# Kyaw-Thiha/animal-vision

Hardware: AMD Instinct MI355X
Metric: megapixels/sec per-frame pipeline (higher is better)
Workload: dtype f16

## Files before the change

### animal-vision_amd/_lib.py

```python
from __future__ import annotations

import ctypes
import os

_HERE = os.path.dirname(os.path.abspath(__file__))
LIB_PATH = os.path.join(_HERE, "libavx.so")

AVX_OK = 0
AVX_ERR_INVALID, AVX_ERR_NO_DEVICE, AVX_ERR_HIP, AVX_ERR_UNSUPPORTED, AVX_ERR_NOMEM = -1, -2, -3, -4, -5
AVX_COLOR_MATRIX, AVX_COLOR_CAT_MERGE = 0, 1
AVX_POST_NONE, AVX_POST_GAUSS, AVX_POST_ROWGAIN, AVX_POST_STREAK = 0, 1, 2, 3
AVX_MAX_KSIZE = 33
AVX_PIX_FMTS = {"yuv420p": 0, "nv12": 1, "yuv422p": 2, "yuv444p": 3, "gray": 4, "yuv420p10le": 5, "yuv422p10le": 6, "yuv444p10le": 7,
                "p010le": 8}
AVX_TRANSFERS = {"pq": 1, "hlg": 2}
AVX_TONEMAPS = {"clip": 0, "mobius": 1}


class AvxError(RuntimeError):
    def __init__(self, code: int, msg: str):
        super().__init__(f"libavx error {code}: {msg}")
        self.code = code


# ... 253 lines not shown
    "avx_yuv_coefficients_d": (_i, [_i, _i, _i, ctypes.POINTER(ctypes.c_int), ctypes.POINTER(ctypes.c_int)]),
    "avx_yuv_frame_size": (_sz, [_i, _i, _i]),
    "avx_yuv_to_rgb_u8": (_i, [_vp, _i, _vp, _vp, _i, _i, _i, _i, _i, _vp]),
    "avx_rgb_to_yuv_u8": (_i, [_vp, _i, _vp, _vp, _i, _i, _i, _i, _i, _vp]),
    "avx_yuv_hdr_to_rgb_u8": (_i, [_vp, _i, _vp, _vp, _i, _i, _i, _i, _i, _i, ctypes.c_double, ctypes.c_double, _vp]),
    "avx_yuv_to_rgb_scaled_u8": (_i, [_vp, _i, _vp, _vp, _i, _i, _i, _i, _i, _i, _i, _vp]),
    "avx_remap_linear_planes": (_i, [_vp, _vp, _i, _i, _i, _vp, _vp, _vp, ctypes.c_float, _vp]),
    "avx_sobel3_plane": (_i, [_vp, _vp, _i, _i, _vp, _vp, _vp]),
    "avx_mst_gram": (_i, [_vp, _vp, _i, _sz, _i, _i, _vp, _vp, _vp, _vp]),
    "avx_mst_qkv_gram": (_i, [_vp, _vp, _vp, _sz, _i, _vp, _vp, _vp, _vp, _vp]),
    "avx_mst_qkv_gram16": (_i, [_vp, _vp, _vp, _sz, _i, _vp, _vp, _vp, _vp, _vp]),
    "avx_mst_ln_gemm_gelu": (_i, [_vp, _vp, _vp, _vp, ctypes.c_float, _vp, _sz, _i, _vp, _vp]),
    "avx_mst_convt2x2": (_i, [_vp, _vp, _vp, _vp, _vp, _i, _i, _i, _i, _vp]),
    "avx_mst_convt2x2_fuse": (_i, [_vp, _vp, _vp, _vp, _vp, _vp, _vp, _i, _i, _i, _i, _vp]),
    "avx_mst_posemb": (_i, [_vp, _vp, _vp, _vp, _vp, _vp, _vp, _i, _i, _i, _i, _vp]),
    "avx_mst_conv3x3_add": (_i, [_vp, _vp, _vp, _vp, _vp, _i, _i, _i, _i, _vp]),
    "avx_mst_attn_pack": (_i, [_vp, _vp, _vp, _vp, _vp, _vp, _i, _vp, _vp]),
    "avx_mst_rowgemm_add": (_i, [_vp, _vp, _vp, _vp, _vp, _vp, _vp, _sz, _i, _vp]),
    "avx_mst_conv_in_u8": (_i, [_vp, _vp, _i, _i, _i, _i, _i, _i, _vp, _vp, _vp]),
    "avx_mst_conv3x3_lds": (_i, [_vp, _vp, _vp, _vp, _vp, _i, _i, _i, _i, _vp]),
    "avx_mst_down4x4": (_i, [_vp, _vp, _vp, _vp, _i, _i, _i, _i, _vp]),
    "avx_mst_conv3x3_lds_gram": (_i, [_vp, _vp, _vp, _vp, _vp, _i, _i, _i, _vp, _vp, _vp, _vp, _vp]),
    "avx_mst_convt2x2_fuse_gram": (_i, [_vp, _vp, _vp, _vp, _vp, _vp, _vp, _i, _i, _i, _vp, _vp, _vp, _vp, _vp]),
    "avx_mst_attn_pack16": (_i, [_vp, _vp, _vp, _vp, _vp, _vp, _i, _vp, _vp]),
    "avx_mst_attn_pack_mx": (_i, [_vp, _vp, _vp, _vp, _vp, _vp, _i, _vp, _vp]),
    "avx_mst_attn_tail_mx": (_i, [_vp, _vp, _vp, _vp, _vp, _vp, _vp, _vp, _i, _i, _i, _i, _vp]),
    "avx_mst_attn_tail": (_i, [_vp, _vp, _vp, _vp, _vp, _vp, _vp, _vp, _i, _i, _i, _i, _vp]),
    "avx_mst_attn_tail_x": (_i, [_vp, _vp, _vp, _vp, _vp, _vp, _vp, _vp, _i, _i, _i, _i, _vp]),
    "avx_mst_ffn_fused": (_i, [_vp, _vp, _vp, _vp, ctypes.c_float, _vp, _vp, _vp, _vp, _i, _i, _i, _i, _vp]),
    "avx_mst_conv3x3_lds_spectral": (_i, [_vp, _vp, _vp, _vp, _i, _i, _i, _fp, _i, _i, _i, _i, _vp, _vp, ctypes.POINTER(ctypes.c_int), _vp]),
    "avx_mst_ffn_fused_mx": (_i, [_vp, _vp, _vp, _vp, ctypes.c_float, _vp, _vp, _vp, _vp, _i, _i, _i, _i, _vp]),
    "avx_mst_gelu_prescale": (ctypes.c_float, []),
    "avx_mst_tile_order": (_i, [_i, _i, _i, _i, _i, ctypes.POINTER(ctypes.c_longlong), _i, ctypes.POINTER(ctypes.c_int)]),
    "avx_mst_dw_gemm_add": (_i, [_vp, _vp, _vp, _vp, _vp, _vp, _i, _i, _i, _i, _vp]),
    "avx_dwconv3x3_nhwc_add": (_i, [_vp, _vp, _vp, _vp, _i, _i, _i, _i, _i, _vp, _vp, _vp]),
    "avx_dwconv3x3_nhwc": (_i, [_vp, _vp, _vp, _vp, _i, _i, _i, _i, _i, _i, _vp]),
    "avx_layernorm_rows": (_i, [_vp, _vp, _vp, _vp, _vp, _i, _sz, _i, ctypes.c_float, _vp]),
    "avx_layernorm_rows_grouped": (_i, [_vp, _vp, _vp, _vp, _vp, _i, _sz, _i, ctypes.c_float, _i, _i, _vp]),
}
for _name, (_res, _args) in _SIGS.items():
    _fn = getattr(lib, _name)
    _fn.restype = _res
    _fn.argtypes = _args

if lib.avx_abi_version() != 1:
    raise ImportError(f"libavx.so ABI {lib.avx_abi_version()} != 1 expected by this package: rebuild")
```

### animal-vision_amd/csrc/mst_fused.hip

```cpp
#include <hip/hip_fp16.h>

#include <cstdio>
#include <cstdlib>
#include <cstring>

#include "avx_internal.h"
#include "mst_common.h"
#include "mst_tile_order.h"

namespace {

typedef float float4_t __attribute__((ext_vector_type(4)));
#ifndef AVX_FFN32_GM2
#define AVX_FFN32_GM2 1
#endif
constexpr int kFT = 512;
constexpr int TS = 16;
constexpr int HS = TS + 2;
#ifndef AVX_FFN_TH
#define AVX_FFN_TH 16
#endif
constexpr int kFfnTH = AVX_FFN_TH;
static_assert(kFfnTH == 14 || kFfnTH == 16, "FeedForward tile rows");
constexpr int kFfnNGRP = (HS * (kFfnTH + 2) + 31) / 32;
// ... 345 lines not shown
#pragma unroll
                    for (int n = 0; n < NT; ++n)
                        D[n] = mfma16(w2f[n * KS2 + s], bf, D[n]);
                }
            }
        }
        stamp(5);
        {
            const int yo = t.y0 + 2 * w8 + (p >> 4), xo = t.x0 + (p & 15);
            if (2 * w8 < FTH && yo < H && xo < W) {
                const size_t off = ((t.b * H + yo) * (size_t)W + xo) * C + 16 * h + 32 * n0;
#pragma unroll
                for (int n = 0; n < NTW; ++n) {
                    const uint4 xa = reinterpret_cast<const uint4*>(x + off + 32 * n)[0], xb = reinterpret_cast<const uint4*>(x + off + 32 * n)[1];
                    const unsigned xw[8] = {xa.x, xa.y, xa.z, xa.w, xb.x, xb.y, xb.z, xb.w};
                    unsigned ow[8];
#pragma unroll
                    for (int j = 0; j < 8; ++j) {
                        float s0 = D[n][2 * j], s1 = D[n][2 * j + 1];
                        fma_mix_lo(s0, xw[j], 0x3c003c00u); fma_mix_hi(s1, xw[j], 0x3c003c00u);
                        ow[j] = pack_f16(s0, s1);
                    }
                    reinterpret_cast<uint4*>(out + off + 32 * n)[0] = uint4{ow[0], ow[1], ow[2], ow[3]};
                    reinterpret_cast<uint4*>(out + off + 32 * n)[1] = uint4{ow[4], ow[5], ow[6], ow[7]};
                }
            }
        }
        stamp(6);
        if (!ahead.live) break;
        t = tile_at(ahead, TS, FTH);
        ahead.advance();
        if (!PREFETCH) fetch(t);
        layernorm();
    }
    if constexpr (STAMP) {
        if (lane == 0 && stamps)
#pragma unroll
            for (int k = 0; k < 8; ++k) stamps[((size_t)blockIdx.x * NW + wave) * 8 + k] = seg[k];
    }
}


constexpr int VS = TS + 4, MS = TS + 2;

template <int C, int MINW>
__global__ __launch_bounds__(kFT, MINW) void k_mst_attn_tail(const __half* __restrict__ v , const __half* __restrict__ x ,
                                                             const uint4* __restrict__ mpack , const __half* __restrict__ taps1 ,
                                                             const __half* __restrict__ taps2 , const float* __restrict__ bias ,
                                                             __half* __restrict__ out, int B, int H, int W, const uint4* __restrict__ wvpack ) {
    constexpr int NO = C / 8, NS = C / 16, NT = C / 32, PP = C * 2 + 16;
    constexpr int VRP = (VS * PP + 255) / 256 * 256, MRP = VRP;
    constexpr int NFILL = (VS * VS * NO + kFT - 1) / kFT;
    extern __shared__ __align__(16) unsigned char smem[];
    unsigned char* vt = smem;
    unsigned char* mt = vt + (size_t)VS * VRP;
    const bool fromx = wvpack != nullptr;
    __half* t2l = reinterpret_cast<__half*>(mt + (size_t)VS * VRP);
    __half* t1l = t2l + 9 * C;
    float* bl = reinterpret_cast<float*>(t1l + 9 * C);
    const int tid = threadIdx.x, lane = tid & 63, wave = tid >> 6, p = lane & 31, h = lane >> 5;
    for (int i = tid; i < 9 * C; i += kFT) { t2l[i] = taps2[i]; t1l[i] = taps1[i]; }
    for (int i = tid; i < C; i += kFT) bl[i] = bias ? bias[i] : 0.f;
    const int tx = (W + TS - 1) / TS, ty = (H + TS - 1) / TS;
    const int oct = wave % NO, part = wave / NO, nparts = 8 / NO, per = (MS * MS + nparts - 1) / nparts;
    half8_t mf[NT * NS];
#pragma unroll
// ... 930 lines not shown
            unsigned o[8];
#pragma unroll
            for (int vv = 0; vv < 8; ++vv) o[vv] = pack_f16(d[2 * vv], d[2 * vv + 1]);
            reinterpret_cast<uint4*>(out + i * 32 + 16 * h)[0] = uint4{o[0], o[1], o[2], o[3]};
            reinterpret_cast<uint4*>(out + i * 32 + 16 * h)[1] = uint4{o[4], o[5], o[6], o[7]};
        }
    }
}

}

static int ffn_fused_launch(avx_ctx* ctx, const void* x, const float* gamma, const float* beta, float eps, const void* w1pack, const void* taps_9xhid, const void* dwpack,
                            const void* w2pack, void* out, int B, int H, int W, int C, void* stream);

extern "C" float avx_mst_gelu_prescale(void) { return kGeluPrescale; }

extern "C" int avx_mst_tile_order(int frames, int ty, int tx, int nwg, int raster, long long* visit, int steps_cap, int* steps_out) {
    if (frames <= 0 || ty <= 0 || tx <= 0 || nwg <= 0 || (visit && steps_cap <= 0) || (long long)frames * ty * tx > 0x7fffffffll) return AVX_ERR_INVALID;
    int most = 0;
    for (int wg = 0; wg < nwg; ++wg) {
        TileWalk wk;
        wk.init((unsigned)wg, (unsigned)nwg, frames, ty, tx, raster ? AVX_TILE_ORDER_RASTER : AVX_TILE_ORDER_XCD);
        int k = 0;
        for (; wk.live; wk.advance(), ++k)
            if (visit && k < steps_cap) visit[(size_t)wg * steps_cap + k] = ((long long)wk.b * ty + wk.yi) * tx + wk.xi;
        if (visit)
            for (int r = k; r < steps_cap; ++r) visit[(size_t)wg * steps_cap + r] = -1;
        most = k > most ? k : most;
    }
    if (steps_out) *steps_out = most;
    return AVX_OK;
}

extern "C" int avx_mst_ffn_fused(avx_ctx* ctx, const void* x, const float* gamma, const float* beta, float eps, const void* w1pack, const void* taps_9xhid,
                                 const void* w2pack, void* out, int B, int H, int W, int C, void* stream) {
    if (!ctx) return AVX_ERR_INVALID;
    AVX_REQUIRE(ctx, taps_9xhid, "avx_mst_ffn_fused: NULL pointer");
    return ffn_fused_launch(ctx, x, gamma, beta, eps, w1pack, taps_9xhid, nullptr, w2pack, out, B, H, W, C, stream);
}

extern "C" int avx_mst_ffn_fused_mx(avx_ctx* ctx, const void* x, const float* gamma, const float* beta, float eps, const void* w1pack, const void* dwpack,
                                    const void* w2pack, void* out, int B, int H, int W, int C, void* stream) {
    if (!ctx) return AVX_ERR_INVALID;
    AVX_REQUIRE(ctx, dwpack && (((uintptr_t)dwpack) & 15u) == 0, "avx_mst_ffn_fused_mx: dwpack NULL or not 16-byte aligned");
    return ffn_fused_launch(ctx, x, gamma, beta, eps, w1pack, nullptr, dwpack, w2pack, out, B, H, W, C, stream);
}

static int ffn_fused_launch(avx_ctx* ctx, const void* x, const float* gamma, const float* beta, float eps, const void* w1pack, const void* taps_9xhid, const void* dwpack,
                            const void* w2pack, void* out, int B, int H, int W, int C, void* stream) {
    AVX_REQUIRE(ctx, x && gamma && beta && w1pack && w2pack && out && B > 0 && H > 0 && W > 0, "avx_mst_ffn_fused: NULL pointer or empty tensor");
    AVX_REQUIRE(ctx, C == 32 || C == 64 || C == 128, "avx_mst_ffn_fused: C=%d (32, 64 or 128: 31-channel groups stored 32 wide)", C);
    AVX_REQUIRE(ctx, ((((uintptr_t)x | (uintptr_t)w1pack | (uintptr_t)w2pack | (uintptr_t)out | (uintptr_t)taps_9xhid)) & 15u) == 0,
                "avx_mst_ffn_fused: pointers must be 16-byte aligned");
    AVX_REQUIRE(ctx, x != out, "avx_mst_ffn_fused: neighbouring tiles read each other's halo: the output cannot be the input");
    AVX_HIP(ctx, hipSetDevice(ctx->device));
    hipStream_t s = avx_pick_stream(ctx, stream);
    const long total = (long)B * ((H + kFfnTH - 1) / kFfnTH) * ((W + TS - 1) / TS);
    const char* hp = getenv("AVX_MST_FFN_HPASS");
    const bool small = C == 32 && !(hp && atoi(hp) == 128);
    const int hpass = (small || C == 128) ? 64 : 128, hpitch = hpass * 2 + 16, rpitch = (HS * hpitch + 255) / 256 * 256;
    const long cap = (long)ctx->num_cus * (small ? 2 : 1);
    const bool nw16 = C == 64 && dwpack && !(getenv("AVX_MST_FFN_NW") && atoi(getenv("AVX_MST_FFN_NW")) == 8);
    const size_t lds = (size_t)kFfnNGRP * 32 * (C * 2 + 16) + (size_t)(kFfnTH + 2) * rpitch + (dwpack ? 0 : (size_t)9 * 4 * C * 2) + sizeof(float) * 2 * C + (nw16 ? (size_t)(C / 32) * (hpass / 16) * 1024 : 0);
    AVX_REQUIRE(ctx, total <= 0x7fffffffl, "avx_mst_ffn_fused: 2^31 tiles or more");
    const dim3 grid((unsigned)(total < cap ? total : cap));
    const int order = mst_tile_order();
#define AVX_FFN1(CV, HP, MW, DW, NWV)                                                                                                            \
    {                                                                                                                                            \
        auto k = k_mst_ffn_fused<CV, HP, MW, DW, false, NWV>;                                                                                    \
        AVX_HIP(ctx, hipFuncSetAttribute((const void*)k, hipFuncAttributeMaxDynamicSharedMemorySize, (int)lds));                                 \
        hipLaunchKernelGGL(k, grid, dim3(64 * NWV), lds, s, (const __half*)x, gamma, beta, eps, (const uint4*)w1pack, (const __half*)taps_9xhid, \
                           (const uint4*)w2pack, (__half*)out, B, H, W, (const uint4*)dwpack, (unsigned long long*)nullptr, order);              \
    }
#define AVX_FFN(CV, HP, MW) { if (dwpack) AVX_FFN1(CV, HP, MW, true, 8) else AVX_FFN1(CV, HP, MW, false, 8) }
    if (dwpack && getenv("AVX_FFN_STAMPS") && ((C == 32 && small) || C == 64 || C == 128)) {
        unsigned long long* d_st = nullptr;
        const int nwv = nw16 ? 16 : 8;
        const size_t n = (size_t)grid.x * nwv * 8;
        AVX_HIP(ctx, hipMalloc((void**)&d_st, n * sizeof(unsigned long long)));
#define AVX_FFN_ST(CV, HP, MW, NWV)                                                                                                              \
    {                                                                                                                                            \
        auto k = k_mst_ffn_fused<CV, HP, MW, true, true, NWV>;                                                                                   \
        AVX_HIP(ctx, hipFuncSetAttribute((const void*)k, hipFuncAttributeMaxDynamicSharedMemorySize, (int)lds));                                 \
        hipLaunchKernelGGL(k, grid, dim3(64 * NWV), lds, s, (const __half*)x, gamma, beta, eps, (const uint4*)w1pack, (const __half*)taps_9xhid, \
                           (const uint4*)w2pack, (__half*)out, B, H, W, (const uint4*)dwpack, d_st, order);                                      \
    }
        if (C == 32) AVX_FFN_ST(32, 64, 4, 8) else if (nw16) AVX_FFN_ST(64, 128, 1, 16) else if (C == 64) AVX_FFN_ST(64, 128, 2, 8) else AVX_FFN_ST(128, 64, 2, 8)
#undef AVX_FFN_ST
        AVX_HIP(ctx, hipStreamSynchronize(s));
        unsigned long long* h_st = (unsigned long long*)malloc(n * sizeof(unsigned long long));
        AVX_HIP(ctx, hipMemcpy(h_st, d_st, n * sizeof(unsigned long long), hipMemcpyDeviceToHost));
        double tot[8] = {0}, w0[8] = {0}, w7[8] = {0};
        for (size_t i = 0; i < n; ++i) { tot[i & 7] += (double)h_st[i]; if (((i >> 3) % nwv) == 0) w0[i & 7] += (double)h_st[i]; if (((i >> 3) % nwv) == (size_t)nwv - 1) w7[i & 7] += (double)h_st[i]; }
        double all = 0;
        for (int k2 = 0; k2 < 8; ++k2) all += tot[k2];
        fprintf(stderr, "[ffn stamps C=%d] %u blocks x %d waves, mean cycles per wave %.0f; share per segment (all waves | first wave | last wave): ", C, grid.x, nwv, all / (grid.x * (double)nwv));
        const char* nm[8] = {"bar1", "phase1", "bar2", "phase2a", "bar3", "phase2b", "epilogue", "ln+fetch"};
        for (int k2 = 0; k2 < 8; ++k2) fprintf(stderr, "%s %.1f%% | %.1f%% | %.1f%%  ", nm[k2], 100 * tot[k2] / all, 100 * w0[k2] * nwv / all, 100 * w7[k2] * nwv / all);
        fprintf(stderr, "\n");
        free(h_st);
        (void)hipFree(d_st);
    } else if (C == 32 && small) AVX_FFN(32, 64, 4) else if (C == 32) AVX_FFN(32, 128, 2)
    else if (nw16) AVX_FFN1(64, 128, 1, true, 16)
    else if (C == 64) AVX_FFN(64, 128, 2) else AVX_FFN(128, 64, 2)
#undef AVX_FFN
#undef AVX_FFN1
    AVX_HIP(ctx, hipGetLastError());
    return AVX_OK;
}

extern "C" int avx_mst_attn_tail(avx_ctx* ctx, const void* v, const void* x, const void* mpack16, const void* taps1_9xc, const void* taps2_9xc, const float* bias,
                                 void* out, int B, int H, int W, int C, void* stream) {
    if (!ctx) return AVX_ERR_INVALID;
    AVX_REQUIRE(ctx, v && x && mpack16 && taps1_9xc && taps2_9xc && out && B > 0 && H > 0 && W > 0, "avx_mst_attn_tail: NULL pointer or empty tensor");
    AVX_REQUIRE(ctx, C == 32 || C == 64, "avx_mst_attn_tail: C=%d (32 or 64)", C);
    AVX_REQUIRE(ctx, ((((uintptr_t)v | (uintptr_t)x | (uintptr_t)mpack16 | (uintptr_t)out | (uintptr_t)taps1_9xc | (uintptr_t)taps2_9xc)) & 15u) == 0,
                "avx_mst_attn_tail: pointers must be 16-byte aligned");
    AVX_REQUIRE(ctx, v != out, "avx_mst_attn_tail: tiles read their neighbours' rows of v: the output cannot be v (it may be x)");
    AVX_HIP(ctx, hipSetDevice(ctx->device));
    hipStream_t s = avx_pick_stream(ctx, stream);
    if (C == 32) return launch_attn_tail<32, 4>(ctx, v, x, mpack16, taps1_9xc, taps2_9xc, bias, out, B, H, W, s, nullptr);
    return launch_attn_tail<64, 2>(ctx, v, x, mpack16, taps1_9xc, taps2_9xc, bias, out, B, H, W, s, nullptr);
}

extern "C" int avx_mst_attn_tail_x(avx_ctx* ctx, const void* x, const void* wvpack16, const void* mpack16, const void* taps1_9xc, const void* taps2_9xc,
                                   const float* bias, void* out, int B, int H, int W, int C, void* stream) {
    if (!ctx) return AVX_ERR_INVALID;
    AVX_REQUIRE(ctx, x && wvpack16 && mpack16 && taps1_9xc && taps2_9xc && out && B > 0 && H > 0 && W > 0, "avx_mst_attn_tail_x: NULL pointer or empty tensor");
    AVX_REQUIRE(ctx, C == 32 || C == 64, "avx_mst_attn_tail_x: C=%d (32 or 64)", C);
    AVX_REQUIRE(ctx, ((((uintptr_t)x | (uintptr_t)wvpack16 | (uintptr_t)mpack16 | (uintptr_t)out | (uintptr_t)taps1_9xc | (uintptr_t)taps2_9xc)) & 15u) == 0,
                "avx_mst_attn_tail_x: pointers must be 16-byte aligned");
    AVX_REQUIRE(ctx, x != out, "avx_mst_attn_tail_x: tiles read their neighbours' rows of x: the output cannot be x");
    AVX_HIP(ctx, hipSetDevice(ctx->device));
    hipStream_t s = avx_pick_stream(ctx, stream);
// ... 133 lines not shown
```

### animal-vision_amd/csrc/mst_tile_order.h

```cpp
#pragma once

#if defined(__HIP_DEVICE_COMPILE__) && __HIP_DEVICE_COMPILE__
#define AVX_TW_UNI32(v) __builtin_amdgcn_readfirstlane((int)(v))
#else
#define AVX_TW_UNI32(v) ((int)(v))
#endif

enum { AVX_TILE_ORDER_RASTER = 0, AVX_TILE_ORDER_XCD = 1 };
constexpr int kTileXcds = 8;

struct TileWalk {
    int xi, yi, b;
    bool live;
    int x1, w;
    int dx, dy, db;
    int tx, ty, nb;
    unsigned per;
    unsigned pos, end, step, stop;

    __host__ __device__ __forceinline__ void locate() {
        const unsigned qb = (unsigned)tx / (unsigned)nb, rb = (unsigned)tx % (unsigned)nb;
        const unsigned wide = rb * (qb + 1) * per;
        unsigned bstart, wv, x0v;
        if (pos < wide) {
// ... 14 lines not shown
        tx = tx_; ty = ty_; per = (unsigned)frames * (unsigned)ty_;
        const unsigned total = per * (unsigned)tx_;
        if (order == AVX_TILE_ORDER_XCD) {
            const unsigned g = wg % kTileXcds, m = wg / kTileXcds, base = nwg / kTileXcds, rem = nwg % kTileXcds;
            const unsigned cum = g * base + (g < rem ? g : rem), n = base + (g < rem ? 1u : 0u);
            nb = tx_ < kTileXcds ? tx_ : kTileXcds;
            pos = (unsigned)AVX_TW_UNI32((unsigned long long)total * cum / nwg) + m;
            end = (unsigned)AVX_TW_UNI32((unsigned long long)total * (cum + n) / nwg);
            step = n;
        } else {
            nb = 1;
            pos = wg; end = total; step = nwg;
        }
        live = pos < end;
        stop = 0;
        if (live) locate();
    }
    __host__ __device__ __forceinline__ void advance() {
        pos += step;
        if (pos >= stop) {
            live = live && pos < end;
            if (live) locate();
            return;
        }
        xi += dx;
        const int cx = xi >= x1 ? 1 : 0;
        xi -= cx ? w : 0;
        yi += dy + cx;
        const int cy = yi >= ty ? 1 : 0;
        yi -= cy ? ty : 0;
        b += db + cy;
    }
};
```

### include/avx.h

```cpp
#ifndef AVX_H
#define AVX_H

#include <stddef.h>
#include <stdint.h>

#ifdef __cplusplus
extern "C" {
#endif

#define AVX_ABI_VERSION 1

typedef struct avx_ctx avx_ctx;

typedef enum avx_status {
    AVX_OK = 0,
    AVX_ERR_INVALID = -1,
    AVX_ERR_NO_DEVICE = -2,
    AVX_ERR_HIP = -3,
    AVX_ERR_UNSUPPORTED = -4,
    AVX_ERR_NOMEM = -5
} avx_status;

int avx_abi_version(void);
int avx_device_count(void);
// ... 268 lines not shown

int avx_mst_conv_in_u8(avx_ctx* ctx, const uint8_t* frame_hwc, int H, int W, int pad_top, int pad_bottom, int pad_left, int pad_right,
                       const float* w_27x32_dev, void* out, void* stream);

int avx_mst_conv3x3_lds(avx_ctx* ctx, const void* x, const void* wpack16, const void* add, void* out, int B, int H, int W, int C, void* stream);
int avx_mst_conv3x3_lds_gram(avx_ctx* ctx, const void* x, const void* wpack16, const void* add, void* out, int H, int W, int C, const void* wqk16, float* gram,
                             float* nq, float* nk, void* stream);
int avx_mst_convt2x2_fuse_gram(avx_ctx* ctx, const void* x, const void* wpack, const float* bias, const void* skip, const void* wskip, void* out, int H, int W, int C,
                               const void* wqk16, float* gram, float* nq, float* nk, void* stream);
int avx_mst_down4x4(avx_ctx* ctx, const void* x, const void* wpack16, void* out, int B, int H, int W, int C, void* stream);

int avx_mst_attn_pack16(avx_ctx* ctx, const float* gram, const float* nq, const float* nk, const float* rescale, const float* wproj_t, int C, void* mpack,
                        void* stream);
int avx_mst_attn_tail(avx_ctx* ctx, const void* v, const void* x, const void* mpack16, const void* taps1_9xc, const void* taps2_9xc, const float* bias,
                      void* out, int B, int H, int W, int C, void* stream);
int avx_mst_attn_tail_x(avx_ctx* ctx, const void* x, const void* wvpack16, const void* mpack16, const void* taps1_9xc, const void* taps2_9xc,
                        const float* bias, void* out, int B, int H, int W, int C, void* stream);
int avx_mst_attn_tail_mx(avx_ctx* ctx, const void* x, const void* wvpack16, const void* mpack_mx, const void* dw1pack, const void* dw2pack,
                         const float* bias, void* out, int B, int H, int W, int C, void* stream);
int avx_mst_attn_pack_mx(avx_ctx* ctx, const float* gram, const float* nq, const float* nk, const float* rescale, const float* wproj_t, int C, void* mpack,
                         void* stream);


int avx_mst_conv3x3_lds_spectral(avx_ctx* ctx, const void* x, const void* wpack16, const void* add, int H, int W, int C, const float* weights_host, int crop_t,
                                 int crop_l, int Hc, int Wc, float* planes_out, void* partials_out, int* n_partials, void* stream);

int avx_mst_ffn_fused(avx_ctx* ctx, const void* x, const float* gamma, const float* beta, float eps, const void* w1pack, const void* taps_9xhid,
                      const void* w2pack, void* out, int B, int H, int W, int C, void* stream);
int avx_mst_ffn_fused_mx(avx_ctx* ctx, const void* x, const float* gamma, const float* beta, float eps, const void* w1pack, const void* dwpack,
                         const void* w2pack, void* out, int B, int H, int W, int C, void* stream);
float avx_mst_gelu_prescale(void);

int avx_mst_tile_order(int frames, int ty, int tx, int nwg, int raster, long long* visit, int steps_cap, int* steps_out);

int avx_mst_rowgemm_add(avx_ctx* ctx, const void* a, const void* wpack, const void* a2, const void* wpack2, const void* add, void* out, size_t rows,
                        int C, void* stream);

int avx_mst_attn_pack(avx_ctx* ctx, const float* gram, const float* nq, const float* nk, const float* rescale, const float* wproj_t, int C,
                      void* mpack, void* stream);

int avx_mst_conv3x3_add(avx_ctx* ctx, const void* x, const void* wpack, const void* add, void* out, int B, int H, int W, int C, void* stream);

int avx_mst_posemb(avx_ctx* ctx, const void* v, const float* w1_c9, const float* w2_c9, const void* residual, const float* bias, void* out, int B,
                   int H, int W, int C, void* stream);

int avx_mst_convt2x2(avx_ctx* ctx, const void* x, const void* wpack, const float* bias, void* out, int B, int H, int W, int C, void* stream);
int avx_mst_convt2x2_fuse(avx_ctx* ctx, const void* x, const void* wpack, const float* bias, const void* skip, const void* wskip, void* out, int B, int H,
                          int W, int C, void* stream);

int avx_dwconv3x3_nhwc(avx_ctx* ctx, const void* x, const float* w_c9, void* y, int dtype, int B, int H, int W, int C, int gelu_out, void* stream);
int avx_dwconv3x3_nhwc_add(avx_ctx* ctx, const void* x, const float* w_c9, void* y, int B, int H, int W, int C, int gelu_out,
                           const void* residual, const float* bias, void* stream);

int avx_layernorm_rows(avx_ctx* ctx, const void* x, const float* gamma, const float* beta, void* y, int dtype, size_t rows, int C, float eps, void* stream);
int avx_layernorm_rows_grouped(avx_ctx* ctx, const void* x, const float* gamma, const float* beta, void* y, int dtype, size_t rows, int C, float eps,
                               int group, int real, void* stream);

int avx_get_table(int which, void* dst_host, size_t capacity);

#ifdef __cplusplus
}
#endif
#endif
```

Measured before the change: 433.0.

## Add column-marching FFN kernel that carries hidden halo rows between vertical steps

Adds a new fused FeedForward kernel in which each workgroup walks down a column of tiles. It stashes the bottom two rows of the GELU'd hidden map in LDS and restores them as the top halo of the next step, so the 1x1 expansion GEMM and LayerNorm are no longer recomputed for halo rows. Only the first step of a column is primed with a full halo computation. The new path is the default for C=32 under XCD tile order and is opt-in for C=64. The trade-offs are more LDS per workgroup for the stash and serialized columns that can leave workgroups unevenly loaded. The stamp-report code is also factored into a shared helper.

```diff
diff --git a/animal-vision_amd/_lib.py b/animal-vision_amd/_lib.py
--- a/animal-vision_amd/_lib.py
+++ b/animal-vision_amd/_lib.py
@@ -309,6 +309,7 @@
     "avx_mst_ffn_fused_mx": (_i, [_vp, _vp, _vp, _vp, ctypes.c_float, _vp, _vp, _vp, _vp, _i, _i, _i, _i, _vp]),
     "avx_mst_gelu_prescale": (ctypes.c_float, []),
     "avx_mst_tile_order": (_i, [_i, _i, _i, _i, _i, ctypes.POINTER(ctypes.c_longlong), _i, ctypes.POINTER(ctypes.c_int)]),
+    "avx_mst_ffn_march_walk": (_i, [_i, _i, _i, _i, ctypes.POINTER(ctypes.c_longlong), ctypes.POINTER(ctypes.c_int), _i, ctypes.POINTER(ctypes.c_int)]),
     "avx_mst_dw_gemm_add": (_i, [_vp, _vp, _vp, _vp, _vp, _vp, _i, _i, _i, _i, _vp]),
     "avx_dwconv3x3_nhwc_add": (_i, [_vp, _vp, _vp, _vp, _i, _i, _i, _i, _i, _vp, _vp, _vp]),
     "avx_dwconv3x3_nhwc": (_i, [_vp, _vp, _vp, _vp, _i, _i, _i, _i, _i, _i, _vp]),
diff --git a/animal-vision_amd/csrc/mst_fused.hip b/animal-vision_amd/csrc/mst_fused.hip
--- a/animal-vision_amd/csrc/mst_fused.hip
+++ b/animal-vision_amd/csrc/mst_fused.hip
@@ -401,6 +401,343 @@
         ahead.advance();
         if (!PREFETCH) fetch(t);
         layernorm();
+    }
+    if constexpr (STAMP) {
+        if (lane == 0 && stamps)
+#pragma unroll
+            for (int k = 0; k < 8; ++k) stamps[((size_t)blockIdx.x * NW + wave) * 8 + k] = seg[k];
+    }
+}
+
+
+template <int C, int HPASS, int MINW, int FTH, bool STAMP = false, int NW = 8>
+__global__ __launch_bounds__(64 * NW, MINW) void k_mst_ffn_march(const __half* __restrict__ x , float eps, const uint4* __restrict__ w1pack ,
+                                                          const uint4* __restrict__ w2pack , __half* __restrict__ out , int B,
+                                                          int H, int W, const uint4* __restrict__ dwpack , unsigned long long* __restrict__ stamps ) {
+    constexpr int HSY = FTH + 2, NNEW = HS * FTH, NGRP = (NNEW + 31) / 32, NPRIME = 2 * HS;
+    constexpr int HID = 4 * C, NPASS = HID / HPASS, KS1 = C / 16, KS2 = HPASS / 16, NT = C / 32, YPITCH = C * 2 + 16, LNV = C / 16;
+    constexpr int HPITCH = HPASS * 2 + 16, RPITCH = (HS * HPITCH + 255) / 256 * 256, NCT = HPASS / 32, SPASS = NPRIME * HPITCH;
+    static_assert(C == 32 || C == 64, "31- or 62-channel blocks (C = 128: eight passes, no room for their stashes)");
+    static_assert(FTH == 14 || FTH == 16, "rows of a step");
+    constexpr int NTHR = 64 * NW, NGW = (NGRP + NW - 1) / NW;
+    constexpr int NTW = NT / (NW / 8), NOCTW = HPASS / (8 * NW);
+    static_assert((NW == 8 || NW == 16) && NT % (NW / 8) == 0 && HPASS % (8 * NW) == 0, "wave split");
+    static_assert(NW >= 2 * NCT * NPASS, "priming: one (pass, group, channel tile) item per wave");
+    constexpr int NCP = NPRIME * (HPASS / 8);
+    static_assert(NCP <= NTHR, "one carried part per thread");
+    extern __shared__ __align__(16) unsigned char smem[];
+    unsigned char* yt = smem;
+    unsigned char* ht = yt + (size_t)NGRP * 32 * YPITCH;
+    unsigned char* stash = ht + (size_t)HSY * RPITCH;
+    constexpr bool W2LDS = NW == 16;
+    uint4* w2l = reinterpret_cast<uint4*>(stash + (size_t)NPASS * SPASS);
+    const int tid = threadIdx.x, lane = tid & 63, wave = tid >> 6, p = lane & 31, h = lane >> 5;
+    unsigned long long seg[8] = {0, 0, 0, 0, 0, 0, 0, 0}, tlast = 0;
+    auto stamp = [&](int k) {
+        if constexpr (STAMP) {
+            const unsigned long long now = __builtin_readcyclecounter();
+            seg[k] += now - tlast;
+            tlast = now;
+        }
+    };
+    if constexpr (STAMP) tlast = __builtin_readcyclecounter();
+    const int tx = (W + TS - 1) / TS, ty = (H + FTH - 1) / FTH;
+    const float cnt = (float)(NT * 31);
+
+    uint4 raw[NGW][LNV];
+    unsigned f_rel[NGW];
+#pragma unroll
+    for (int gi = 0; gi < NGW; ++gi) {
+        const int q = 32 * (wave + NW * gi) + p, qq = q < NNEW ? q : NNEW - 1;
+        f_rel[gi] = (unsigned)(((qq / HS) * W + qq % HS) * C + h * (C / 2)) * 2u;
+    }
+    auto new_inside = [&](const Tile& t) { return t.y0 + HSY - 1 <= H && t.x0 >= 1 && t.x0 + HS - 1 <= W; };
+    auto fetch = [&](const Tile& t) {
+        if (new_inside(t)) {
+            const char* origin = reinterpret_cast<const char*>(x + ((t.b * H + t.y0 + 1) * (size_t)W + t.x0 - 1) * C);
+#pragma unroll
+            for (int gi = 0; gi < NGW; ++gi) {
+                if (wave + NW * gi >= NGRP) break;
+                unsigned o = f_rel[gi];
+                asm volatile("" : "+v"(o));
+                const uint4* src = reinterpret_cast<const uint4*>(origin + o);
+#pragma unroll
+                for (int v = 0; v < LNV; ++v) raw[gi][v] = src[v];
+            }
+            return;
+        }
+#pragma unroll
+        for (int gi = 0; gi < NGW; ++gi) {
+            const int g = wave + NW * gi;
+            if (g >= NGRP) break;
+            const int q = 32 * g + p, qq = q < NNEW ? q : NNEW - 1;
+            int yy = t.y0 + 1 + qq / HS, xx = t.x0 - 1 + qq % HS;
+            yy = yy >= H ? H - 1 : yy;
+            xx = xx < 0 ? 0 : (xx >= W ? W - 1 : xx);
+            const uint4* src = reinterpret_cast<const uint4*>(x + ((t.b * H + yy) * (size_t)W + xx) * C + h * (C / 2));
+#pragma unroll
+            for (int v = 0; v < LNV; ++v) raw[gi][v] = src[v];
+        }
+    };
+    auto ln_group = [&](const uint4 (&rw)[LNV], unsigned char* yb, int g) {
+        typedef _Float16 half2v __attribute__((ext_vector_type(2)));
+        constexpr unsigned kOnes = 0x3c003c00u;
+        auto is_pad = [&](int i) { return ((h * (C / 2) + i) & 31) == 31; };
+        auto word = [&](int i) { const uint4 u = rw[i / 8]; const int k = (i / 2) & 3; return k == 0 ? u.x : k == 1 ? u.y : k == 2 ? u.z : u.w; };
+        float s1 = 0.f;
+#pragma unroll
+        for (int i = 0; i < 8 * LNV; i += 2) s1 = __builtin_amdgcn_fdot2(__builtin_bit_cast(half2v, word(i)), __builtin_bit_cast(half2v, kOnes), s1, false);
+        const float mean = (s1 + __shfl_xor(s1, 32)) / cnt, nmean = -mean;
+        float d[8 * LNV], s2 = 0.f;
+#pragma unroll
+        for (int i = 0; i < 8 * LNV; ++i) {
+            const float t = (i & 1) ? fma_mix_hi_c(word(i), kOnes, nmean) : fma_mix_lo_c(word(i), kOnes, nmean);
+            d[i] = is_pad(i) ? 0.f : t;
+            s2 = __builtin_fmaf(d[i], d[i], s2);
+        }
+        const float rstd = rsqrtf((s2 + __shfl_xor(s2, 32)) / cnt + eps);
+        unsigned char* dst = yb + (size_t)(32 * g + p) * YPITCH + h * C;
+#pragma unroll
+        for (int v = 0; v < LNV; ++v) {
+            unsigned o[4];
+#pragma unroll
+            for (int j = 0; j < 8; j += 2) {
+                const int i = 8 * v + j;
+                const float2_t y2 = float2_t{d[i], d[i + 1]} * float2_t{rstd, rstd};
+                const float bq = (h * (C / 2) + i + 1) == 31 ? 1.0f : y2.y;
+                o[j / 2] = pack_f16(y2.x, bq);
+            }
+            *reinterpret_cast<uint4*>(dst + 16 * v) = uint4{o[0], o[1], o[2], o[3]};
+        }
+    };
+    auto layernorm = [&]() {
+#pragma unroll
+        for (int gi = 0; gi < NGW; ++gi) {
+            if (wave + NW * gi >= NGRP) break;
+            ln_group(raw[gi], yt, wave + NW * gi);
+        }
+    };
+    auto p1_item = [&](const half8_t (&wf)[KS1], const unsigned char* yb, int g, unsigned char* dst, bool store, bool masked, uint32_t keep) {
+        float16_t d;
+#pragma unroll
+        for (int v = 0; v < 16; ++v) d[v] = 0.f;
+        const unsigned char* ysrc = yb + (size_t)(32 * g + p) * YPITCH + 16 * h;
+#pragma unroll
+        for (int s = 0; s < KS1; ++s) d = mfma16(wf[s], __builtin_bit_cast(half8_t, *reinterpret_cast<const uint4*>(ysrc + 32 * s)), d);
+        if (store) {
+            constexpr int GP1 = C == 32 ? 2 : 1;
+            unsigned pk[8];
+#pragma unroll
+            for (int v0 = 0; v0 < 8; v0 += GP1) {
+                float2_t gq[GP1];
+#pragma unroll
+                for (int v = 0; v < GP1; ++v) gq[v] = float2_t{d[2 * (v0 + v)], d[2 * (v0 + v) + 1]};
+                gelu_mx<GP1>(gq);
+#pragma unroll
+                for (int v = 0; v < GP1; ++v) pk[v0 + v] = pack_f16(gq[v].x, gq[v].y);
+            }
+            uint4 u0 = uint4{pk[0], pk[1], pk[2], pk[3]}, u1 = uint4{pk[4], pk[5], pk[6], pk[7]};
+            if (masked) { u0.x &= keep; u0.y &= keep; u0.z &= keep; u0.w &= keep; u1.x &= keep; u1.y &= keep; u1.z &= keep; u1.w &= keep; }
+            reinterpret_cast<uint4*>(dst)[0] = u0;
+            reinterpret_cast<uint4*>(dst)[1] = u1;
+        }
+    };
+    auto carry = [&](int pass, bool save) {
+        if (tid < NCP) {
+            int i = tid;
+            asm volatile("" : "+v"(i));
+            const int pix = i / (HPASS / 8), part = i % (HPASS / 8), r = pix / HS, c = pix % HS;
+            uint4* m = reinterpret_cast<uint4*>(ht + (size_t)(r + (save ? FTH : 0)) * RPITCH + (size_t)c * HPITCH + 16 * part);
+            uint4* s = reinterpret_cast<uint4*>(stash + (size_t)pass * SPASS + (size_t)pix * HPITCH + 16 * part);
+            if (save) *s = *m; else *m = *s;
+        }
+    };
+
+    const int n0 = (wave / 8) * NTW, w8 = wave % 8;
+    half8_t w2f[W2LDS ? 1 : NTW * KS2];
+    auto load_w2 = [&](int pass) {
+#pragma unroll
+        for (int n = 0; n < NTW; ++n)
+#pragma unroll
+            for (int s = 0; s < KS2; ++s) w2f[n * KS2 + s] = __builtin_bit_cast(half8_t, w2pack[((size_t)(n0 + n) * (HID / 16) + pass * KS2 + s) * 64 + lane]);
+    };
+    if constexpr (NPASS == 1 && !W2LDS) load_w2(0);
+    if constexpr (NPASS == 1 && W2LDS)
+        for (int i = tid; i < NT * KS2 * 64; i += NTHR) w2l[i] = w2pack[((size_t)(i / (KS2 * 64)) * (HID / 16) + (i / 64) % KS2) * 64 + (i & 63)];
+    constexpr int NITEM = (NGRP + NW / NCT - 1) / (NW / NCT);
+    int p1_g[NITEM], p1_dst[NITEM], p1_yx[NITEM];
+#pragma unroll
+    for (int j = 0; j < NITEM; ++j) {
+        const int g = wave / NCT + j * (NW / NCT), q = 32 * g + p, qc = q < NNEW ? q : 0;
+        p1_g[j] = g < NGRP ? g : -1;
+        p1_dst[j] = (g < NGRP && q < NNEW) ? (2 + qc / HS) * RPITCH + (qc % HS) * HPITCH + 32 * h : -1;
+        p1_yx[j] = ((qc / HS + 1) << 16) | (qc % HS);
+    }
+    MarchWalk ahead;
+    ahead.init(blockIdx.x, gridDim.x, B, ty, tx);
+    if (!ahead.live) return;
+    Tile t = Tile{ahead.xi * TS, ahead.si * FTH, (long)ahead.b};
+    bool prime = ahead.prime;
+    ahead.advance();
+    fetch(t);
+    for (;;) {
+        layernorm();
+        if (prime) {
+            unsigned char* yp = ht + (size_t)FTH * RPITCH;
+            int pp = p, wv = wave;
+            asm volatile("" : "+v"(pp), "+v"(wv));
+            static_assert(64 * YPITCH <= 2 * RPITCH, "the primed rows' LayerNorm fits two map rows");
+            if (wv < 2) {
+                const int q = 32 * wv + pp, qq = q < NPRIME ? q : NPRIME - 1;
+                int yy = t.y0 - 1 + qq / HS, xx = t.x0 - 1 + qq % HS;
+                yy = yy < 0 ? 0 : (yy >= H ? H - 1 : yy);
+                xx = xx < 0 ? 0 : (xx >= W ? W - 1 : xx);
+                const uint4* src = reinterpret_cast<const uint4*>(x + ((t.b * H + yy) * (size_t)W + xx) * C + h * (C / 2));
+                uint4 rp[LNV];
+#pragma unroll
+                for (int v = 0; v < LNV; ++v) rp[v] = src[v];
+                ln_group(rp, yp, wv);
+            }
+            __syncthreads();
+            if (wv < 2 * NCT * NPASS) {
+                const int pass = wv / (2 * NCT), g = (wv / NCT) % 2, ct = wv % NCT, q = 32 * g + pp;
+                half8_t wf[KS1];
+#pragma unroll
+                for (int s = 0; s < KS1; ++s) wf[s] = __builtin_bit_cast(half8_t, w1pack[((size_t)(pass * NCT + ct) * KS1 + s) * 64 + lane]);
+                const int qc = q < NPRIME ? q : 0, yy = t.y0 - 1 + qc / HS, xx = t.x0 - 1 + qc % HS;
+                const uint32_t keep = (yy >= 0 && yy < H && xx >= 0 && xx < W) ? 0xffffffffu : 0u;
+                p1_item(wf, yp, g, stash + (size_t)pass * SPASS + (size_t)qc * HPITCH + 32 * h + 64 * ct, q < NPRIME, true, keep);
+            }
+        }
+        const bool inside = new_inside(t);
+        float16_t D[NTW];
+#pragma unroll
+        for (int n = 0; n < NTW; ++n)
+#pragma unroll
+            for (int v = 0; v < 16; ++v) D[n][v] = 0.f;
+#pragma unroll 1
+        for (int pass = 0; pass < NPASS; ++pass) {
+            stamp(pass == 0 ? 7 : 5);
+            __syncthreads();
+            stamp(0);
+            if constexpr (W2LDS && NPASS > 1)
+                for (int i = tid; i < NT * KS2 * 64; i += NTHR) w2l[i] = w2pack[((size_t)(i / (KS2 * 64)) * (HID / 16) + pass * KS2 + (i / 64) % KS2) * 64 + (i & 63)];
+            half8_t af[NOCTW][3];
+#pragma unroll
+            for (int o2 = 0; o2 < NOCTW; ++o2)
+#pragma unroll
+                for (int i = 0; i < 3; ++i) af[o2][i] = __builtin_bit_cast(half8_t, dwpack[((size_t)(pass * (HPASS / 8) + NW * o2 + wave) * 3 + i) * 64 + lane]);
+            {
+                const int ct = wave % NCT;
+                half8_t w1f[KS1];
+#pragma unroll
+                for (int s = 0; s < KS1; ++s) w1f[s] = __builtin_bit_cast(half8_t, w1pack[((size_t)(pass * NCT + ct) * KS1 + s) * 64 + lane]);
+                carry(pass, false);
+#pragma unroll
+                for (int j = 0; j < NITEM; ++j) {
+                    if (p1_g[j] < 0) continue;
+                    uint32_t keep = 0xffffffffu;
+                    if (!inside) {
+                        const int yy = t.y0 + (p1_yx[j] >> 16), xx = t.x0 + (p1_yx[j] & 0xffff) - 1;
+                        keep = (yy < H && xx >= 0 && xx < W) ? 0xffffffffu : 0u;
+                    }
+                    p1_item(w1f, yt, p1_g[j], ht + p1_dst[j] + 64 * ct, p1_dst[j] >= 0, !inside, keep);
+                }
+            }
+            stamp(1);
+            __syncthreads();
+            stamp(2);
+            if (pass == NPASS - 1 && ahead.live) fetch(Tile{ahead.xi * TS, ahead.si * FTH, (long)ahead.b});
+            if constexpr (NPASS > 1 && !W2LDS) load_w2(pass);
+            carry(pass, true);
+            const int n16 = lane & 15, q = lane >> 4;
+            unsigned char* rbase = ht + (size_t)q * RPITCH + (size_t)n16 * HPITCH + 16 * wave;
+            unsigned char* wbase = ht + (size_t)(q >> 1) * RPITCH + (size_t)n16 * HPITCH + 16 * wave + 8 * (q & 1);
+            constexpr int NU = NOCTW * (FTH / 2);
+            uint4 bq[3];
+            auto rd = [&](int u) {
+                const int o2 = u / (FTH / 2), pr = u % (FTH / 2);
+#pragma unroll
+                for (int i = 0; i < 3; ++i) bq[i] = *reinterpret_cast<const uint4*>(rbase + (size_t)(2 * pr) * RPITCH + (size_t)i * HPITCH + 16 * NW * o2);
+            };
+            auto finish = [&](int u, float4_t a) {
+                const int o2 = u / (FTH / 2), pr = u % (FTH / 2);
+                float2_t gp[2] = {float2_t{a[0], a[1]}, float2_t{a[2], a[3]}};
+                if constexpr (C == 64 || (C == 32 && AVX_FFN32_GM2)) gelu_mx<2>(gp);
+                else { float2_t g0[1] = {gp[0]}, g1[1] = {gp[1]}; gelu_mx<1>(g0); gelu_mx<1>(g1); gp[0] = g0[0]; gp[1] = g1[0]; }
+                *reinterpret_cast<uint2*>(wbase + (size_t)(2 * pr) * RPITCH + 16 * NW * o2) = uint2{pack_f16(gp[0].x, gp[0].y), pack_f16(gp[1].x, gp[1].y)};
+            };
+            constexpr bool PIPE = C == 64 || AVX_FFN_PIPE_ALL;
+            if constexpr (PIPE) {
+                rd(0);
+                float4_t prev = {0.f, 0.f, 0.f, 0.f};
+#pragma unroll
+                for (int u = 0; u < NU; ++u) {
+                    const int o2 = u / (FTH / 2);
+                    float4_t acc = {0.f, 0.f, 0.f, 0.f};
+#pragma unroll
+                    for (int i = 0; i < 3; ++i) acc = __builtin_amdgcn_mfma_f32_16x16x32_f16(af[o2][i], __builtin_bit_cast(half8_t, bq[i]), acc, 0, 0, 0);
+                    if (u + 1 < NU) rd(u + 1);
+                    __builtin_amdgcn_sched_barrier(0);
+                    if (u > 0) finish(u - 1, prev);
+                    __builtin_amdgcn_sched_barrier(0);
+                    prev = acc;
+                }
+                finish(NU - 1, prev);
+            } else {
+#pragma unroll
+                for (int u = 0; u < NU; ++u) {
+                    const int o2 = u / (FTH / 2);
+                    rd(u);
+                    float4_t acc = {0.f, 0.f, 0.f, 0.f};
+#pragma unroll
+                    for (int i = 0; i < 3; ++i) acc = __builtin_amdgcn_mfma_f32_16x16x32_f16(af[o2][i], __builtin_bit_cast(half8_t, bq[i]), acc, 0, 0, 0);
+                    finish(u, acc);
+                }
+            }
+            stamp(3);
+            __syncthreads();
+            stamp(4);
+            if (2 * w8 < FTH) {
+                const int r = 2 * w8 + (p >> 4), c = p & 15;
+                const unsigned char* zb = ht + (size_t)r * RPITCH + (size_t)c * HPITCH + 16 * h;
+#pragma unroll
+                for (int s = 0; s < KS2; ++s) {
+                    const half8_t bf = __builtin_bit_cast(half8_t, *reinterpret_cast<const uint4*>(zb + 32 * s));
+#pragma unroll
+                    for (int n = 0; n < NTW; ++n) {
+                        if constexpr (W2LDS) D[n] = mfma16(__builtin_bit_cast(half8_t, w2l[((n0 + n) * KS2 + s) * 64 + lane]), bf, D[n]);
+                        else D[n] = mfma16(w2f[n * KS2 + s], bf, D[n]);
+                    }
+                }
+            }
+        }
+        stamp(5);
+        {
+            const int yo = t.y0 + 2 * w8 + (p >> 4), xo = t.x0 + (p & 15);
+            if (2 * w8 < FTH && yo < H && xo < W) {
+                const size_t off = ((t.b * H + yo) * (size_t)W + xo) * C + 16 * h + 32 * n0;
+#pragma unroll
+                for (int n = 0; n < NTW; ++n) {
+                    const uint4 xa = reinterpret_cast<const uint4*>(x + off + 32 * n)[0], xb = reinterpret_cast<const uint4*>(x + off + 32 * n)[1];
+                    const unsigned xw[8] = {xa.x, xa.y, xa.z, xa.w, xb.x, xb.y, xb.z, xb.w};
+                    unsigned ow[8];
+#pragma unroll
+                    for (int j = 0; j < 8; ++j) {
+                        float s0 = D[n][2 * j], s1 = D[n][2 * j + 1];
+                        fma_mix_lo(s0, xw[j], 0x3c003c00u); fma_mix_hi(s1, xw[j], 0x3c003c00u);
+                        ow[j] = pack_f16(s0, s1);
+                    }
+                    reinterpret_cast<uint4*>(out + off + 32 * n)[0] = uint4{ow[0], ow[1], ow[2], ow[3]};
+                    reinterpret_cast<uint4*>(out + off + 32 * n)[1] = uint4{ow[4], ow[5], ow[6], ow[7]};
+                }
+            }
+        }
+        stamp(6);
+        if (!ahead.live) break;
+        t = Tile{ahead.xi * TS, ahead.si * FTH, (long)ahead.b};
+        prime = ahead.prime;
+        ahead.advance();
     }
     if constexpr (STAMP) {
         if (lane == 0 && stamps)
@@ -1397,6 +1734,28 @@
     return AVX_OK;
 }
 
+extern "C" int avx_mst_ffn_march_walk(int frames, int ty, int tx, int nwg, long long* visit, int* prime, int steps_cap, int* steps_out) {
+    if (frames <= 0 || ty <= 0 || tx <= 0 || nwg <= 0 || ((visit || prime) && steps_cap <= 0) || (long long)frames * ty * tx > 0x7fffffffll) return AVX_ERR_INVALID;
+    int most = 0;
+    for (int wg = 0; wg < nwg; ++wg) {
+        MarchWalk wk;
+        wk.init((unsigned)wg, (unsigned)nwg, frames, ty, tx);
+        int k = 0;
+        for (; wk.live; wk.advance(), ++k)
+            if (k < steps_cap) {
+                if (visit) visit[(size_t)wg * steps_cap + k] = ((long long)wk.b * tx + wk.xi) * ty + wk.si;
+                if (prime) prime[(size_t)wg * steps_cap + k] = wk.prime ? 1 : 0;
+            }
+        for (int r = k; r < steps_cap; ++r) {
+            if (visit) visit[(size_t)wg * steps_cap + r] = -1;
+            if (prime) prime[(size_t)wg * steps_cap + r] = -1;
+        }
+        most = k > most ? k : most;
+    }
+    if (steps_out) *steps_out = most;
+    return AVX_OK;
+}
+
 extern "C" int avx_mst_ffn_fused(avx_ctx* ctx, const void* x, const float* gamma, const float* beta, float eps, const void* w1pack, const void* taps_9xhid,
                                  const void* w2pack, void* out, int B, int H, int W, int C, void* stream) {
     if (!ctx) return AVX_ERR_INVALID;
@@ -1409,6 +1768,64 @@
     if (!ctx) return AVX_ERR_INVALID;
     AVX_REQUIRE(ctx, dwpack && (((uintptr_t)dwpack) & 15u) == 0, "avx_mst_ffn_fused_mx: dwpack NULL or not 16-byte aligned");
     return ffn_fused_launch(ctx, x, gamma, beta, eps, w1pack, nullptr, dwpack, w2pack, out, B, H, W, C, stream);
+}
+
+static int ffn_stamps_report(avx_ctx* ctx, const char* what, int C, unsigned blocks, int nwv, unsigned long long* d_st) {
+    const size_t n = (size_t)blocks * nwv * 8;
+    unsigned long long* h_st = (unsigned long long*)malloc(n * sizeof(unsigned long long));
+    AVX_HIP(ctx, hipMemcpy(h_st, d_st, n * sizeof(unsigned long long), hipMemcpyDeviceToHost));
+    double tot[8] = {0}, w0[8] = {0}, w7[8] = {0};
+    for (size_t i = 0; i < n; ++i) { tot[i & 7] += (double)h_st[i]; if (((i >> 3) % nwv) == 0) w0[i & 7] += (double)h_st[i]; if (((i >> 3) % nwv) == (size_t)nwv - 1) w7[i & 7] += (double)h_st[i]; }
+    double all = 0;
+    for (int k2 = 0; k2 < 8; ++k2) all += tot[k2];
+    fprintf(stderr, "[%s C=%d] %u blocks x %d waves, mean cycles per wave %.0f; share per segment (all waves | first wave | last wave): ", what, C, blocks, nwv, all / (blocks * (double)nwv));
+    const char* nm[8] = {"bar1", "phase1", "bar2", "phase2a", "bar3", "phase2b", "epilogue", "ln+fetch"};
+    for (int k2 = 0; k2 < 8; ++k2) fprintf(stderr, "%s %.1f%% | %.1f%% | %.1f%%  ", nm[k2], 100 * tot[k2] / all, 100 * w0[k2] * nwv / all, 100 * w7[k2] * nwv / all);
+    fprintf(stderr, "\n");
+    free(h_st);
+    return AVX_OK;
+}
+
+constexpr int kMarchRows = 14;
+static bool ffn_marches(int C, bool dwpack, bool small, bool nw16, int order) {
+    if (!dwpack || order != AVX_TILE_ORDER_XCD || !((C == 32 && small) || (C == 64 && nw16))) return false;
+    const char* e = getenv("AVX_MST_FFN_MARCH");
+    if (!e) return C == 32;
+    return !strcmp(e, "all") || atoi(e) == C;
+}
+
+static int ffn_march_launch(avx_ctx* ctx, const void* x, float eps, const void* w1pack, const void* dwpack, const void* w2pack, void* out, int B, int H, int W, int C, hipStream_t s) {
+    const bool c32 = C == 32;
+    constexpr int rows = kMarchRows;
+    const int hpass = c32 ? 64 : 128, hpitch = hpass * 2 + 16, rpitch = (HS * hpitch + 255) / 256 * 256, nwv = c32 ? 8 : 16;
+    const long total = (long)B * ((H + rows - 1) / rows) * ((W + TS - 1) / TS);
+    AVX_REQUIRE(ctx, total <= 0x7fffffffl, "avx_mst_ffn_fused_mx: 2^31 steps or more");
+    long cap = (long)ctx->num_cus * (c32 ? 2 : 1);
+    const char* wg = getenv("AVX_MST_FFN_WGS");
+    if (wg && atol(wg) > 0 && atol(wg) < cap) cap = atol(wg);
+    const dim3 grid((unsigned)(total < cap ? total : cap));
+    const size_t lds = (size_t)((HS * rows + 31) / 32) * 32 * (C * 2 + 16) + (size_t)(rows + 2) * rpitch + (size_t)(4 * C / hpass) * 2 * HS * hpitch + (c32 ? 0 : (size_t)(C / 32) * (hpass / 16) * 1024);
+    unsigned long long* d_st = nullptr;
+    const bool st = getenv("AVX_FFN_STAMPS") != nullptr;
+    if (st) AVX_HIP(ctx, hipMalloc((void**)&d_st, (size_t)grid.x * nwv * 8 * sizeof(unsigned long long)));
+#define AVX_FFN_MARCH(CV, HP, MW, TH, ST, NWV)                                                                                                          \
+    {                                                                                                                                                   \
+        auto k = k_mst_ffn_march<CV, HP, MW, TH, ST, NWV>;                                                                                              \
+        AVX_HIP(ctx, hipFuncSetAttribute((const void*)k, hipFuncAttributeMaxDynamicSharedMemorySize, (int)lds));                                        \
+        hipLaunchKernelGGL(k, grid, dim3(64 * NWV), lds, s, (const __half*)x, eps, (const uint4*)w1pack, (const uint4*)w2pack, (__half*)out, B, H, W,    \
+                           (const uint4*)dwpack, d_st);                                                                                                 \
+    }
+    if (c32) { if (st) AVX_FFN_MARCH(32, 64, 4, kMarchRows, true, 8) else AVX_FFN_MARCH(32, 64, 4, kMarchRows, false, 8) }
+    else { if (st) AVX_FFN_MARCH(64, 128, 1, kMarchRows, true, 16) else AVX_FFN_MARCH(64, 128, 1, kMarchRows, false, 16) }
+#undef AVX_FFN_MARCH
+    AVX_HIP(ctx, hipGetLastError());
+    if (st) {
+        AVX_HIP(ctx, hipStreamSynchronize(s));
+        const int rc = ffn_stamps_report(ctx, "ffn march stamps", C, grid.x, nwv, d_st);
+        (void)hipFree(d_st);
+        return rc;
+    }
+    return AVX_OK;
 }
 
 static int ffn_fused_launch(avx_ctx* ctx, const void* x, const float* gamma, const float* beta, float eps, const void* w1pack, const void* taps_9xhid, const void* dwpack,
@@ -1430,6 +1847,7 @@
     AVX_REQUIRE(ctx, total <= 0x7fffffffl, "avx_mst_ffn_fused: 2^31 tiles or more");
     const dim3 grid((unsigned)(total < cap ? total : cap));
     const int order = mst_tile_order();
+    if (ffn_marches(C, dwpack != nullptr, small, nw16, order)) return ffn_march_launch(ctx, x, eps, w1pack, dwpack, w2pack, out, B, H, W, C, s);
 #define AVX_FFN1(CV, HP, MW, DW, NWV)                                                                                                            \
     {                                                                                                                                            \
         auto k = k_mst_ffn_fused<CV, HP, MW, DW, false, NWV>;                                                                                    \
@@ -1453,18 +1871,9 @@
         if (C == 32) AVX_FFN_ST(32, 64, 4, 8) else if (nw16) AVX_FFN_ST(64, 128, 1, 16) else if (C == 64) AVX_FFN_ST(64, 128, 2, 8) else AVX_FFN_ST(128, 64, 2, 8)
 #undef AVX_FFN_ST
         AVX_HIP(ctx, hipStreamSynchronize(s));
-        unsigned long long* h_st = (unsigned long long*)malloc(n * sizeof(unsigned long long));
-        AVX_HIP(ctx, hipMemcpy(h_st, d_st, n * sizeof(unsigned long long), hipMemcpyDeviceToHost));
-        double tot[8] = {0}, w0[8] = {0}, w7[8] = {0};
-        for (size_t i = 0; i < n; ++i) { tot[i & 7] += (double)h_st[i]; if (((i >> 3) % nwv) == 0) w0[i & 7] += (double)h_st[i]; if (((i >> 3) % nwv) == (size_t)nwv - 1) w7[i & 7] += (double)h_st[i]; }
-        double all = 0;
-        for (int k2 = 0; k2 < 8; ++k2) all += tot[k2];
-        fprintf(stderr, "[ffn stamps C=%d] %u blocks x %d waves, mean cycles per wave %.0f; share per segment (all waves | first wave | last wave): ", C, grid.x, nwv, all / (grid.x * (double)nwv));
-        const char* nm[8] = {"bar1", "phase1", "bar2", "phase2a", "bar3", "phase2b", "epilogue", "ln+fetch"};
-        for (int k2 = 0; k2 < 8; ++k2) fprintf(stderr, "%s %.1f%% | %.1f%% | %.1f%%  ", nm[k2], 100 * tot[k2] / all, 100 * w0[k2] * nwv / all, 100 * w7[k2] * nwv / all);
-        fprintf(stderr, "\n");
-        free(h_st);
+        const int rc = ffn_stamps_report(ctx, "ffn stamps", C, grid.x, nwv, d_st);
         (void)hipFree(d_st);
+        if (rc != AVX_OK) return rc;
     } else if (C == 32 && small) AVX_FFN(32, 64, 4) else if (C == 32) AVX_FFN(32, 128, 2)
     else if (nw16) AVX_FFN1(64, 128, 1, true, 16)
     else if (C == 64) AVX_FFN(64, 128, 2) else AVX_FFN(128, 64, 2)
diff --git a/animal-vision_amd/csrc/mst_tile_order.h b/animal-vision_amd/csrc/mst_tile_order.h
--- a/animal-vision_amd/csrc/mst_tile_order.h
+++ b/animal-vision_amd/csrc/mst_tile_order.h
@@ -70,3 +70,32 @@
         b += db + cy;
     }
 };
+
+struct MarchWalk {
+    int si, xi, b;
+    bool live, prime;
+    int ty, tx;
+    unsigned pos, end;
+
+    __host__ __device__ __forceinline__ void init(unsigned wg, unsigned nwg, int frames, int ty_, int tx_) {
+        ty = ty_; tx = tx_;
+        const unsigned long long total = (unsigned long long)frames * (unsigned)ty_ * (unsigned)tx_;
+        pos = (unsigned)AVX_TW_UNI32(total * wg / nwg);
+        end = (unsigned)AVX_TW_UNI32(total * (wg + 1ull) / nwg);
+        live = pos < end;
+        prime = true;
+        const unsigned col = pos / (unsigned)ty_, fr = col / (unsigned)tx_;
+        si = AVX_TW_UNI32(pos - col * (unsigned)ty_); xi = AVX_TW_UNI32(col - fr * (unsigned)tx_); b = AVX_TW_UNI32(fr);
+    }
+    __host__ __device__ __forceinline__ void advance() {
+        ++pos;
+        live = pos < end;
+        ++si;
+        prime = si >= ty;
+        if (prime) {
+            si = 0;
+            ++xi;
+            if (xi >= tx) { xi = 0; ++b; }
+        }
+    }
+};
diff --git a/include/avx.h b/include/avx.h
--- a/include/avx.h
+++ b/include/avx.h
@@ -324,6 +324,7 @@
 float avx_mst_gelu_prescale(void);
 
 int avx_mst_tile_order(int frames, int ty, int tx, int nwg, int raster, long long* visit, int steps_cap, int* steps_out);
+int avx_mst_ffn_march_walk(int frames, int ty, int tx, int nwg, long long* visit, int* prime, int steps_cap, int* steps_out);
 
 int avx_mst_rowgemm_add(avx_ctx* ctx, const void* a, const void* wpack, const void* a2, const void* wpack2, const void* add, void* out, size_t rows,
                         int C, void* stream);
```

New measurement: 436.6, median of 3. About the same (+0.8%).
